# facebookresearch/PointContrast

Measured on AMD Instinct MI355X. Metric: scene-pairs/sec, ScanNet 2.5cm Res16UNet34C PointInfoNCE, higher is better.
Workload: dtype f32; 1 GPU; BASELINE configs[1]: Res16UNet34C, nce loss, voxel 0.025 m, 4 pairs/GPU, 87380+87371 active voxels per forward pair on rank 0, npos 4096, T 0.4, SGD(lr 0.1, mom 0.8, wd 1e-4); global_batch=4, parallelism=dp1, engine=native, pair_execution=one two-segment pass (BatchNorm statistics per cloud)

## Files before the change

pointcontrast_amd/csrc/spconv_wgrad_x3.hip:

```cpp
#include <algorithm>
#include <cstdio>
#include <cstdlib>
#include <type_traits>

#include "common.h"
#include "internal.h"
#include "x3_split.h"

namespace pcmi {

struct WgradTArgs {
  const float* x;
  int64_t x_ld;
  const float* g;
  int64_t g_ld;
  const int32_t* nbr;
  const int32_t* perm;
  int64_t n_rows;
  int K, C, N;
  int RB, NG;
  int tiles_per_rb;
  float* slabs;
};

template <int MTW, int NTW, int KG, int TERMS>
__global__ __launch_bounds__(256, 2) void wgrad_x3t_kernel(WgradTArgs a) {
  constexpr int TR = 64, RG = TR / 8;
  constexpr int CB = 32 * MTW, NB = 32 * NTW;
  constexpr uint32_t kAbsent = 0x80000000u;
  constexpr int kRsrcFlags = 0x00020000;
  __shared__ __attribute__((aligned(16))) u32x4 s_x[TERMS * RG * CB];
  __shared__ __attribute__((aligned(16))) u32x4 s_g[TERMS * RG * NB];
  __shared__ uint32_t s_xoff[KG][TR];
  __shared__ uint32_t s_goff[TR];
  __shared__ int s_any[KG];

  const int t = threadIdx.x, lane = t & 63, wave = t >> 6;
  const int i = lane & 15, kk = lane >> 4;
  const int wm = wave >> 1, wn = wave & 1;
  const int b = blockIdx.x;
  const int og = (b >> 3) % a.NG;
  const int rb = (b & 7) + 8 * (b / (8 * a.NG));
  const int kbase = og * KG;
  const int c0 = blockIdx.y * CB, n0 = blockIdx.z * NB;
  const int n_tiles = (int)((a.n_rows + TR - 1) / TR);
  const int t0 = rb * a.tiles_per_rb, t1 = min(t0 + a.tiles_per_rb, n_tiles);
  const __amdgpu_buffer_rsrc_t xr = __builtin_amdgcn_make_buffer_rsrc(const_cast<float*>(a.x), 0, 0x7FFFFFFF, kRsrcFlags);
  const __amdgpu_buffer_rsrc_t gr = __builtin_amdgcn_make_buffer_rsrc(const_cast<float*>(a.g), 0, 0x7FFFFFFF, kRsrcFlags);
  const uint32_t xld = (uint32_t)(a.x_ld * 4), gld = (uint32_t)(a.g_ld * 4);

  f32x4 acc[KG][MTW][NTW];
#pragma unroll
  for (int s = 0; s < KG; ++s)
#pragma unroll
    for (int mt = 0; mt < MTW; ++mt)
#pragma unroll
      for (int nt = 0; nt < NTW; ++nt) acc[s][mt][nt] = (f32x4){0.f, 0.f, 0.f, 0.f};

  const int rg_s = t & 7, q_s = t >> 3;
  auto stage = [&](u32x4* dst, const __amdgpu_buffer_rsrc_t& rsrc, const uint32_t* offs, int ch0, int width) {
    if (q_s < width / 4) {
      v4f v[8];
      const uint32_t col = (uint32_t)(ch0 + 4 * q_s) * 4u;
#pragma unroll
      for (int e = 0; e < 8; ++e)
        v[e] = __builtin_bit_cast(v4f, __builtin_amdgcn_raw_buffer_load_b128(rsrc, offs[8 * rg_s + e] + col, 0, 0));
#pragma unroll
      for (int e4 = 0; e4 < 4; ++e4) {
        const v4f x0 = {v[0][e4], v[1][e4], v[2][e4], v[3][e4]}, x1 = {v[4][e4], v[5][e4], v[6][e4], v[7][e4]};
        u32x4 h, m, l;
        split_terms<TERMS>(x0, x1, h, m, l);
        const int cell = rg_s * width + ((4 * q_s + e4) ^ rg_s);
        dst[cell] = h;
        if constexpr (TERMS == 3) {
          dst[RG * width + cell] = m;
          dst[2 * RG * width + cell] = l;
        }
      }
    }
  };

  for (int tile = t0; tile < t1; ++tile) {
    const int64_t p0 = (int64_t)tile * TR;
    __syncthreads();
    if (t < TR) {
      const int64_t pos = p0 + t;
      uint32_t o = kAbsent;
      if (pos < a.n_rows) o = (uint32_t)(a.perm ? a.perm[pos] : (int32_t)pos) * gld;
      s_goff[t] = o;
    }
    for (int idx = t; idx < KG * TR; idx += 256) {
      const int s = idx >> 6, rr = idx & 63, k = kbase + s;
      const int64_t pos = p0 + rr;
      int32_t v = -1;
      if (k < a.K && pos < a.n_rows) v = a.nbr ? a.nbr[(int64_t)k * a.n_rows + pos] : (int32_t)pos;
      s_xoff[s][rr] = v >= 0 ? (uint32_t)v * xld : kAbsent;
      const bool any = __ballot(v >= 0) != 0ull;
      if (lane == 0) s_any[s] = any ? 1 : 0;
    }
    __syncthreads();
    bool any_k = false;
#pragma unroll
    for (int s = 0; s < KG; ++s) any_k |= s_any[s] != 0;
    if (!any_k) continue;
    stage(s_g, gr, s_goff, n0, NB);
#pragma unroll
    for (int s = 0; s < KG; ++s) {
      if (s_any[s] == 0) continue;
      stage(s_x, xr, s_xoff[s], c0, CB);
      __syncthreads();
#pragma unroll
      for (int step = 0; step < TR / 32; ++step) {
        const int rgq = 4 * step + kk;
        u32x4 ah[MTW], am[MTW], al[MTW];
#pragma unroll
        for (int mt = 0; mt < MTW; ++mt) {
          const int cell = rgq * CB + ((16 * (wm * MTW + mt) + i) ^ rgq);
          ah[mt] = s_x[cell];
          if constexpr (TERMS == 3) {
            am[mt] = s_x[RG * CB + cell];
            al[mt] = s_x[2 * RG * CB + cell];
          }
        }
#pragma unroll
        for (int nt = 0; nt < NTW; ++nt) {
          const int cell = rgq * NB + ((16 * (wn * NTW + nt) + i) ^ rgq);
          const u32x4 bh = s_g[cell];
          u32x4 bm, bl;
          if constexpr (TERMS == 3) {
            bm = s_g[RG * NB + cell];
            bl = s_g[2 * RG * NB + cell];
          }
#define PCMI_WX3_MFMA(AT, BT)                                                                                              \
  acc[s][mt][nt] = __builtin_amdgcn_mfma_f32_16x16x32_bf16(__builtin_bit_cast(bf16x8, AT[mt]), __builtin_bit_cast(bf16x8, BT), \
                                                           acc[s][mt][nt], 0, 0, 0)
#pragma unroll
          for (int mt = 0; mt < MTW; ++mt) {
            if constexpr (TERMS == 3) {
              PCMI_WX3_MFMA(al, bh);
              PCMI_WX3_MFMA(ah, bl);
              PCMI_WX3_MFMA(am, bm);
              PCMI_WX3_MFMA(am, bh);
              PCMI_WX3_MFMA(ah, bm);
            }
            PCMI_WX3_MFMA(ah, bh);
          }
#undef PCMI_WX3_MFMA
        }
      }
      __syncthreads();
    }
  }

#pragma unroll
  for (int s = 0; s < KG; ++s) {
    const int k = kbase + s;
    if (k >= a.K) continue;
    float* slab = a.slabs + ((int64_t)k * a.RB + rb) * a.C * a.N;
#pragma unroll
    for (int mt = 0; mt < MTW; ++mt)
#pragma unroll
      for (int nt = 0; nt < NTW; ++nt)
#pragma unroll
        for (int r = 0; r < 4; ++r) {
          const int c = c0 + 16 * (wm * MTW + mt) + 4 * kk + r, n = n0 + 16 * (wn * NTW + nt) + i;
          slab[(int64_t)c * a.N + n] = acc[s][mt][nt][r];
        }
  }
}

template <int MTW, int NTW, int KG>
__global__ __launch_bounds__(512, 2) void wgrad_x3p_kernel(WgradTArgs a) {
  static_assert(KG % 2 == 0 && KG >= 2 && KG <= 4, "slot parity = offset parity; one producer wave per offset slot");
  constexpr int TR = 64, RG = TR / 8;
  constexpr int CB = 32 * MTW, NB = 32 * NTW;
  constexpr uint32_t kAbsent = 0x80000000u;
  constexpr int kRsrcFlags = 0x00020000;
  __shared__ __attribute__((aligned(16))) u32x4 s_x[2][3 * RG * CB];
  __shared__ __attribute__((aligned(16))) u32x4 s_g[2][3 * RG * NB];
  __shared__ uint32_t s_xoff[3][KG][TR];
  __shared__ uint32_t s_goff[3][TR];
  __shared__ int s_any[3][KG];

  const int t = threadIdx.x, lane = t & 63;
  const int wave = __builtin_amdgcn_readfirstlane(t >> 6);
  const bool producer = wave >= 4;
  const int b = blockIdx.x;
  const int og = (b >> 3) % a.NG;
  const int rb = (b & 7) + 8 * (b / (8 * a.NG));
  const int kbase = og * KG;
  const int c0 = blockIdx.y * CB, n0 = blockIdx.z * NB;
  const int n_tiles = (int)((a.n_rows + TR - 1) / TR);
  const int t0 = rb * a.tiles_per_rb, t1 = min(t0 + a.tiles_per_rb, n_tiles);
  const int nt_tiles = max(t1 - t0, 0);
  const uint32_t xld = (uint32_t)(a.x_ld * 4), gld = (uint32_t)(a.g_ld * 4);

  if (producer) {
    const __amdgpu_buffer_rsrc_t xr = __builtin_amdgcn_make_buffer_rsrc(const_cast<float*>(a.x), 0, 0x7FFFFFFF, kRsrcFlags);
    const __amdgpu_buffer_rsrc_t gr = __builtin_amdgcn_make_buffer_rsrc(const_cast<float*>(a.g), 0, 0x7FFFFFFF, kRsrcFlags);
    const int pt = t - 256;
    int32_t tab_v[(KG + 3) / 4];
    int32_t tab_g = -1;
    auto table_issue = [&](int tl) {
      const int64_t p0 = (int64_t)(t0 + tl) * TR;
      const bool in_range = tl < nt_tiles;
      const int64_t pos = p0 + lane;
#pragma unroll
      for (int j = 0; j < (KG + 3) / 4; ++j) {
        const int sx = wave - 4 + 4 * j, k = kbase + sx;
        tab_v[j] = -1;
        if (sx < KG && in_range && k < a.K && pos < a.n_rows) tab_v[j] = a.nbr ? a.nbr[(int64_t)k * a.n_rows + pos] : (int32_t)pos;
      }
      tab_g = -1;
      if (wave == 4 && in_range && pos < a.n_rows) tab_g = a.perm ? a.perm[pos] : (int32_t)pos;
    };
    auto table_commit = [&](int tl) {
      const int sl = tl % 3;
#pragma unroll
      for (int j = 0; j < (KG + 3) / 4; ++j) {
        const int sx = wave - 4 + 4 * j;
        if (sx < KG) {
          s_xoff[sl][sx][lane] = tab_v[j] >= 0 ? (uint32_t)tab_v[j] * xld : kAbsent;
          const bool any = __ballot(tab_v[j] >= 0) != 0ull;
          if (lane == 0) s_any[sl][sx] = any ? 1 : 0;
        }
      }
      if (wave == 4) s_goff[sl][lane] = tab_g >= 0 ? (uint32_t)tab_g * gld : kAbsent;
    };
    const int rg_s = pt & 7, q_s = pt >> 3;
    auto issue = [&](auto& v, const __amdgpu_buffer_rsrc_t& rsrc, const uint32_t* offs, int ch0, auto wtag, auto e0tag, auto e1tag) {
      constexpr int W = decltype(wtag)::value, CPT = W / 32, E0 = decltype(e0tag)::value, E1 = decltype(e1tag)::value;
      const uint32_t col = (uint32_t)(ch0 + CPT * q_s) * 4u;
#pragma unroll
      for (int e = E0; e < E1; ++e) {
        const uint32_t o = offs[8 * rg_s + e] + col;
        if constexpr (CPT == 3) {
          const auto t3 = __builtin_amdgcn_raw_buffer_load_b96(rsrc, o, 0, 0);
          static_assert(sizeof(t3) >= 12, "b96");
          __builtin_memcpy(&v[e], &t3, 12);
        } else {
          const auto t2 = __builtin_amdgcn_raw_buffer_load_b64(rsrc, o, 0, 0);
          static_assert(sizeof(t2) == 8, "b64");
          __builtin_memcpy(&v[e], &t2, 8);
        }
      }
    };
    auto finish = [&](u32x4* dst, const auto& v, auto wtag, auto c0tag, auto c1tag) {
      constexpr int W = decltype(wtag)::value, CPT = W / 32, EC0 = decltype(c0tag)::value, EC1 = decltype(c1tag)::value;
#pragma unroll
      for (int ec = EC0; ec < (EC1 < CPT ? EC1 : CPT); ++ec) {
        const v4f x0 = {v[0].f[ec], v[1].f[ec], v[2].f[ec], v[3].f[ec]}, x1 = {v[4].f[ec], v[5].f[ec], v[6].f[ec], v[7].f[ec]};
        u32x4 h, m, l;
        split3(x0, x1, h, m, l);
        const int cell = rg_s * W + ((CPT * q_s + ec) ^ rg_s);
        dst[cell] = h;
        dst[RG * W + cell] = m;
        dst[2 * RG * W + cell] = l;
      }
    };
    struct Row { float f[3]; };
    constexpr std::integral_constant<int, CB> kWX{};
    constexpr std::integral_constant<int, NB> kWG{};
    constexpr std::integral_constant<int, 0> k0{};
    constexpr std::integral_constant<int, 8> k8{};
    static_assert(KG == 4, "one register set per offset slot");
    Row r0[8], r1[8], r2[8], r3[8], rgv[8];
    table_issue(0);
    table_commit(0);
    table_issue(1);
    table_commit(1);
    __syncthreads();
    issue(r0, xr, s_xoff[0][0], c0, kWX, k0, k8);
    issue(rgv, gr, s_goff[0], n0, kWG, k0, k8);
    issue(r1, xr, s_xoff[0][1], c0, kWX, k0, k8);
    issue(r2, xr, s_xoff[0][2], c0, kWX, k0, k8);
    finish(s_x[0], r0, kWX, k0, k8);
    finish(s_g[0], rgv, kWG, k0, k8);
    issue(rgv, gr, s_goff[1], n0, kWG, k0, k8);
    __syncthreads();
#define PCMI_X3P_SET(j) ((j) == 0 ? r0 : ((j) == 1 ? r1 : ((j) == 2 ? r2 : r3)))
    for (int tl = 0; tl < nt_tiles; ++tl) {
#pragma unroll
      for (int sx = 0; sx < KG; ++sx) {
        if (sx == 0) table_issue(tl + 2);
        {
          const int s3 = (sx + 3) % KG, tl3 = tl + (sx + 3) / KG;
          issue(PCMI_X3P_SET(s3), xr, s_xoff[tl3 % 3][s3], c0, kWX, k0, k8);
        }
        finish(s_x[(sx + 1) & 1], PCMI_X3P_SET((sx + 1) % KG), kWX, k0, k8);
        if (sx == 1) finish(s_g[(tl + 1) & 1], rgv, kWG, k0, k8);
        if (sx == KG - 2) table_commit(tl + 2);
        if (sx == KG - 1) issue(rgv, gr, s_goff[(tl + 2) % 3], n0, kWG, k0, k8);
        __syncthreads();
      }
    }
#undef PCMI_X3P_SET
    return;
  }

  const int i = lane & 15, kk = lane >> 4;
  const int wm = wave >> 1, wn = wave & 1;
  f32x4 acc[KG][MTW][NTW];
#pragma unroll
  for (int sx = 0; sx < KG; ++sx)
#pragma unroll
    for (int mt = 0; mt < MTW; ++mt)
#pragma unroll
      for (int nt = 0; nt < NTW; ++nt) acc[sx][mt][nt] = (f32x4){0.f, 0.f, 0.f, 0.f};
  __syncthreads();
  __syncthreads();
  for (int tl = 0; tl < nt_tiles; ++tl) {
    const u32x4* sg = s_g[tl & 1];
#pragma unroll
    for (int sx = 0; sx < KG; ++sx) {
      if (s_any[tl % 3][sx] != 0) {
        const u32x4* sxp = s_x[sx & 1];
        u32x4 ah[MTW], am[MTW], al[MTW];
        u32x4 bh[2], bm[2], bl[2];
        auto read_a = [&](int step) {
          const int rgq = 4 * step + kk;
#pragma unroll
          for (int mt = 0; mt < MTW; ++mt) {
            const int cell = rgq * CB + ((16 * (wm * MTW + mt) + i) ^ rgq);
            ah[mt] = sxp[cell];
            am[mt] = sxp[RG * CB + cell];
            al[mt] = sxp[2 * RG * CB + cell];
          }
        };
        auto read_b = [&](int step, int nt, int slot) {
          const int rgq = 4 * step + kk;
          const int cell = rgq * NB + ((16 * (wn * NTW + nt) + i) ^ rgq);
          bh[slot] = sg[cell];
          bm[slot] = sg[RG * NB + cell];
          bl[slot] = sg[2 * RG * NB + cell];
        };
        constexpr int STEPS = TR / 32;
        read_a(0);
        read_b(0, 0, 0);
        __builtin_amdgcn_sched_barrier(0);
#pragma unroll
        for (int it = 0; it < STEPS * NTW; ++it) {
          const int step = it / NTW, nt = it % NTW, slot = it & 1;
          if (it + 1 < STEPS * NTW) read_b((it + 1) / NTW, (it + 1) % NTW, slot ^ 1);
          __builtin_amdgcn_sched_barrier(0);
#define PCMI_WX3P_MFMA(AT, BT)                                                                                                      \
  acc[sx][mt][nt] = __builtin_amdgcn_mfma_f32_16x16x32_bf16(__builtin_bit_cast(bf16x8, AT[mt]), __builtin_bit_cast(bf16x8, BT[slot]), \
                                                            acc[sx][mt][nt], 0, 0, 0)
#pragma unroll
          for (int mt = 0; mt < MTW; ++mt) {
            PCMI_WX3P_MFMA(al, bh);
            PCMI_WX3P_MFMA(ah, bl);
            PCMI_WX3P_MFMA(am, bm);
            PCMI_WX3P_MFMA(am, bh);
            PCMI_WX3P_MFMA(ah, bm);
            PCMI_WX3P_MFMA(ah, bh);
          }
#undef PCMI_WX3P_MFMA
          __builtin_amdgcn_sched_barrier(0);
          if (nt == NTW - 1 && step + 1 < STEPS) {
            read_a(step + 1);
            __builtin_amdgcn_sched_barrier(0);
          }
        }
      }
      __syncthreads();
    }
  }
#pragma unroll
  for (int sx = 0; sx < KG; ++sx) {
    const int k = kbase + sx;
    if (k >= a.K) continue;
    float* slab = a.slabs + ((int64_t)k * a.RB + rb) * a.C * a.N;
#pragma unroll
    for (int mt = 0; mt < MTW; ++mt)
#pragma unroll
      for (int nt = 0; nt < NTW; ++nt)
#pragma unroll
        for (int r = 0; r < 4; ++r) {
          const int c = c0 + 16 * (wm * MTW + mt) + 4 * kk + r, n = n0 + 16 * (wn * NTW + nt) + i;
          slab[(int64_t)c * a.N + n] = acc[sx][mt][nt][r];
        }
  }
}


__global__ __launch_bounds__(256) void wgrad_slab_sum_kernel(const float* __restrict__ slabs, int RB, int64_t per_k,
                                                             float* __restrict__ gw, int accumulate) {
  __shared__ float s_part[8][33];
  const int k = blockIdx.y;
  const int el = threadIdx.x & 31, cl = threadIdx.x >> 5;
  const int64_t e = (int64_t)blockIdx.x * 32 + el;
  float s = 0.f;
  if (e < per_k)
    for (int r = cl; r < RB; r += 8) s += slabs[((int64_t)k * RB + r) * per_k + e];
  s_part[cl][el] = s;
  __syncthreads();
  if (cl != 0 || e >= per_k) return;
#pragma unroll
  for (int q = 1; q < 8; ++q) s += s_part[q][el];
  float* dst = gw + (int64_t)k * per_k + e;
  *dst = accumulate ? *dst + s : s;
}

constexpr int kWgradTKG = 4;
constexpr int kWgradTMaxRB = 128;

static int wgrad_x3t_tw(int c) { return c % 96 == 0 ? 3 : (c % 64 == 0 ? 2 : 0); }

static int64_t wgrad_x3t_min_rows() {
  const char* e = getenv("PCMI_WGRAD_X3T");
  return e ? (int64_t)atoll(e) : (int64_t)8192;
}

static bool wgrad_x3t_dense_on() {
  const char* e = getenv("PCMI_WGRAD_X3T_DENSE");
  return !(e && e[0] == '0');
}

bool wgrad_x3t_eligible(const pcmi_kmap_t* map, int64_t n_in, int64_t n_out, int cin, int cout, int64_t in_ld, int64_t gout_ld) {
  const int64_t mr = wgrad_x3t_min_rows();
  const bool shape = map ? (map->kernel_size == 3 && map->stride == 1) : wgrad_x3t_dense_on();
  return shape && mr > 0 && n_out >= mr && n_in == n_out && cin >= 64 && cout >= 64 &&
         wgrad_x3t_tw(cin) > 0 && wgrad_x3t_tw(cout) > 0 && n_in * in_ld * 4 <= 0x7FFFFF00ll && n_out * gout_ld * 4 <= 0x7FFFFF00ll;
}

static int wgrad_x3p_mode() {
  const char* e = getenv("PCMI_WGRAD_X3P");
  return e ? (atoi(e) != 0 ? 1 : 0) : 1;
}

static int wgrad_x3t_rb(int64_t n_rows, int gy, int gz, int per_cu = 2, int K = PCMI_MAX_KERNEL_VOLUME, int kg = kWgradTKG) {
  const int NG = (K + kg - 1) / kg;
  const int64_t n_tiles = ceil_div(n_rows, 64);
  int64_t rb = (int64_t)per_cu * num_cu() / ((int64_t)NG * gy * gz);
  rb = std::min<int64_t>(rb, n_tiles / 4);
  rb = std::max<int64_t>(8, std::min<int64_t>(kWgradTMaxRB, rb / 8 * 8));
  return (int)rb;
}

size_t wgrad_x3t_workspace(int64_t n_rows, int cin, int cout) {
  const int MTW = wgrad_x3t_tw(cin), NTW = wgrad_x3t_tw(cout);
  const int64_t mr = wgrad_x3t_min_rows();
  if (MTW == 0 || NTW == 0 || mr <= 0 || n_rows < mr || cin < 64 || cout < 64) return 0;
  return (size_t)PCMI_MAX_KERNEL_VOLUME * wgrad_x3t_rb(n_rows, cin / (32 * MTW), cout / (32 * NTW)) * cin * cout * sizeof(float);
}

template <int MTW, int NTW>
static void launch_x3t(const WgradTArgs& a, dim3 grid, int mode, int terms, hipStream_t st) {
  if (terms == 1) wgrad_x3t_kernel<MTW, NTW, kWgradTKG, 1><<<grid, 256, 0, st>>>(a);
  else if (mode == 1) wgrad_x3p_kernel<MTW, NTW, kWgradTKG><<<grid, 512, 0, st>>>(a);
  else wgrad_x3t_kernel<MTW, NTW, kWgradTKG, 3><<<grid, 256, 0, st>>>(a);
}

int wgrad_x3t_run(const float* in, int64_t in_ld, const float* gout, int64_t gout_ld, int64_t n_rows, int cin, int cout,
                  const pcmi_kmap_t* map, float* gweight, int accumulate, void* ws, size_t ws_bytes, hipStream_t st) {
  const int MTW = wgrad_x3t_tw(cin), NTW = wgrad_x3t_tw(cout);
  PCMI_REQUIRE(MTW > 0 && NTW > 0 && (!map || map->K <= PCMI_MAX_KERNEL_VOLUME), PCMI_ERR_UNSUPPORTED, "wgrad x3t: channels (%d, %d)", cin, cout);
  WgradTArgs a;
  a.x = in;
  a.x_ld = in_ld;
  a.g = gout;
  a.g_ld = gout_ld;
  a.nbr = !map ? nullptr : ((map->perm && map->nbr_perm) ? map->nbr_perm : map->nbr);
  a.perm = (map && map->perm && map->nbr_perm) ? map->perm : nullptr;
  a.n_rows = n_rows;
  const int K = map ? map->K : 1;
  a.K = K;
  a.C = cin;
  a.N = cout;
  const int gy = cin / (32 * MTW), gz = cout / (32 * NTW);
  const int terms = conv_terms();
  const int mode = terms == 1 ? 0 : wgrad_x3p_mode();
  [[maybe_unused]] const bool pc = mode == 1;
  const int kg = kWgradTKG;
  a.NG = (K + kg - 1) / kg;
  a.RB = wgrad_x3t_rb(n_rows, gy, gz, mode >= 1 ? 1 : 2, K, kg);
  a.tiles_per_rb = (int)ceil_div(ceil_div(n_rows, 64), a.RB);
  const size_t need = (size_t)K * a.RB * cin * cout * sizeof(float);
  PCMI_REQUIRE(ws && ws_bytes >= need, PCMI_ERR_WORKSPACE, "wgrad x3t: workspace %zu < %zu bytes", ws_bytes, need);
  a.slabs = (float*)ws;
  const dim3 grid((unsigned)(a.RB * a.NG), (unsigned)gy, (unsigned)gz);
  switch (MTW * 4 + NTW) {
    case 3 * 4 + 3: launch_x3t<3, 3>(a, grid, mode, terms, st); break;
    case 3 * 4 + 2: launch_x3t<3, 2>(a, grid, mode, terms, st); break;
    case 2 * 4 + 3: launch_x3t<2, 3>(a, grid, mode, terms, st); break;
    default: launch_x3t<2, 2>(a, grid, mode, terms, st); break;
  }
  PCMI_LAUNCH_CHECK();
  const int64_t per_k = (int64_t)cin * cout;
  wgrad_slab_sum_kernel<<<dim3((unsigned)ceil_div(per_k, 32), (unsigned)K), 256, 0, st>>>(a.slabs, a.RB, per_k, gweight, accumulate);
  PCMI_LAUNCH_CHECK();
  return PCMI_OK;
}

}
```

Measured before the change: 294.7 scene-pairs/sec.

## Move gradient-tile loads and split from producer waves to MFMA consumer waves

The gathered gradient (g) tile loading and its three-way float split are moved off the producer waves and onto the 256 consumer (MFMA) threads. Loads are issued in rounds and interleaved across offset slots with two register sets. Producer waves now only stream x rows, which shortens the producer critical path per slot. In exchange, consumer waves take on extra VGPR pressure and memory latency between MFMA phases, which could reduce overlap or occupancy.

```diff
diff --git a/pointcontrast_amd/csrc/spconv_wgrad_x3.hip b/pointcontrast_amd/csrc/spconv_wgrad_x3.hip
--- a/pointcontrast_amd/csrc/spconv_wgrad_x3.hip
+++ b/pointcontrast_amd/csrc/spconv_wgrad_x3.hip
@@ -197,7 +197,6 @@
 
   if (producer) {
     const __amdgpu_buffer_rsrc_t xr = __builtin_amdgcn_make_buffer_rsrc(const_cast<float*>(a.x), 0, 0x7FFFFFFF, kRsrcFlags);
-    const __amdgpu_buffer_rsrc_t gr = __builtin_amdgcn_make_buffer_rsrc(const_cast<float*>(a.g), 0, 0x7FFFFFFF, kRsrcFlags);
     const int pt = t - 256;
     int32_t tab_v[(KG + 3) / 4];
     int32_t tab_g = -1;
@@ -260,23 +259,19 @@
     };
     struct Row { float f[3]; };
     constexpr std::integral_constant<int, CB> kWX{};
-    constexpr std::integral_constant<int, NB> kWG{};
     constexpr std::integral_constant<int, 0> k0{};
     constexpr std::integral_constant<int, 8> k8{};
     static_assert(KG == 4, "one register set per offset slot");
-    Row r0[8], r1[8], r2[8], r3[8], rgv[8];
+    Row r0[8], r1[8], r2[8], r3[8];
     table_issue(0);
     table_commit(0);
     table_issue(1);
     table_commit(1);
     __syncthreads();
     issue(r0, xr, s_xoff[0][0], c0, kWX, k0, k8);
-    issue(rgv, gr, s_goff[0], n0, kWG, k0, k8);
     issue(r1, xr, s_xoff[0][1], c0, kWX, k0, k8);
     issue(r2, xr, s_xoff[0][2], c0, kWX, k0, k8);
     finish(s_x[0], r0, kWX, k0, k8);
-    finish(s_g[0], rgv, kWG, k0, k8);
-    issue(rgv, gr, s_goff[1], n0, kWG, k0, k8);
     __syncthreads();
 #define PCMI_X3P_SET(j) ((j) == 0 ? r0 : ((j) == 1 ? r1 : ((j) == 2 ? r2 : r3)))
     for (int tl = 0; tl < nt_tiles; ++tl) {
@@ -288,9 +283,7 @@
           issue(PCMI_X3P_SET(s3), xr, s_xoff[tl3 % 3][s3], c0, kWX, k0, k8);
         }
         finish(s_x[(sx + 1) & 1], PCMI_X3P_SET((sx + 1) % KG), kWX, k0, k8);
-        if (sx == 1) finish(s_g[(tl + 1) & 1], rgv, kWG, k0, k8);
         if (sx == KG - 2) table_commit(tl + 2);
-        if (sx == KG - 1) issue(rgv, gr, s_goff[(tl + 2) % 3], n0, kWG, k0, k8);
         __syncthreads();
       }
     }
@@ -307,7 +300,33 @@
     for (int mt = 0; mt < MTW; ++mt)
 #pragma unroll
       for (int nt = 0; nt < NTW; ++nt) acc[sx][mt][nt] = (f32x4){0.f, 0.f, 0.f, 0.f};
+  static_assert(NTW + 1 <= KG && NTW <= 3, "round r is converted in slot r + 1; two register sets");
+  const __amdgpu_buffer_rsrc_t gr = __builtin_amdgcn_make_buffer_rsrc(const_cast<float*>(a.g), 0, 0x7FFFFFFF, kRsrcFlags);
+  float ga[8], gb[8];
+  const int rg_g = t >> 5, q_g = t & 31;
+  auto g_issue = [&](float (&v)[8], const uint32_t* offs, int r) {
+    const uint32_t col = (uint32_t)(n0 + q_g) * 4u;
+#pragma unroll
+    for (int e = 0; e < 8; ++e)
+      v[e] = __builtin_bit_cast(float, __builtin_amdgcn_raw_buffer_load_b32(gr, offs[8 * rg_g + e] + col + 128u * r, 0, 0));
+  };
+  auto g_finish = [&](u32x4* dst, const float (&v)[8], int r) {
+    const v4f x0 = {v[0], v[1], v[2], v[3]}, x1 = {v[4], v[5], v[6], v[7]};
+    u32x4 h, m, l;
+    split3(x0, x1, h, m, l);
+    const int cell = rg_g * NB + (q_g ^ rg_g) + 32 * r;
+    dst[cell] = h;
+    dst[RG * NB + cell] = m;
+    dst[2 * RG * NB + cell] = l;
+  };
   __syncthreads();
+  g_issue(ga, s_goff[0], 0);
+  g_issue(gb, s_goff[0], 1);
+  g_finish(s_g[0], ga, 0);
+  if constexpr (NTW == 3) g_issue(ga, s_goff[0], 2);
+  g_finish(s_g[0], gb, 1);
+  if constexpr (NTW == 3) g_finish(s_g[0], ga, 2);
+  g_issue(ga, s_goff[1], 0);
   __syncthreads();
   for (int tl = 0; tl < nt_tiles; ++tl) {
     const u32x4* sg = s_g[tl & 1];
@@ -363,6 +382,10 @@
           }
         }
       }
+      if (sx >= 1 && sx <= NTW) g_finish(s_g[(tl + 1) & 1], sx == 2 ? gb : ga, sx - 1);
+      if (sx == 0) g_issue(gb, s_goff[(tl + 1) % 3], 1);
+      if (sx == 1 && NTW == 3) g_issue(ga, s_goff[(tl + 1) % 3], 2);
+      if (sx == KG - 1) g_issue(ga, s_goff[(tl + 2) % 3], 0);
       __syncthreads();
     }
   }
```

After: 297.9 scene-pairs/sec (median of 6 runs). 1.1% higher.
